# georghess/neurad-studio

Hardware: AMD Instinct MI355X
Metric: ray-samples/sec (4096 rays x 128 samples) (higher is better)
Workload: dtype f32; 1 GPU; BASELINE config[1]: NeuRAD hash-grid (16 levels, T=2^19, F=2, fp32) + 64-wide MLPs, 4096 rays x 128 samples per GPU, PowerSampler bins + ray ordering pass + fused field + compositing (forward / render path); rays_per_gpu=4096, samples_per_ray=128, parallelism=rays sharded x1, no collective

## Files before the change

neurad_studio_amd/csrc/render.hip:

```cpp
#include "common.h"
#include "render_variants.h"

namespace nrhip {

struct FieldDev {
  GridDev grid;
  const void* table;
  float scale;
  const float* gw0; const float* gb0;
  const float* gw1; const float* gb1;
  const float* fw0; const float* fb0;
  const float* fw1; const float* fb1;
  const float* fw2; const float* fb2;
  int use_sdf;
  float beta;
  uint32_t lay[NRHIP_MAX_LEVELS * 4];
};

struct SaveDev {
  float* enc;
  float* hg;
  float* xf;
  float* hf;
};

template <int H, Prod PROD = Prod::F32>
struct Lds {
  static constexpr int NB = H / 16;
  static constexpr int WS(int n) { return PROD == Prod::Bf16Split ? n + n / 2 : n; }
  static constexpr int G0 = 0;
  static constexpr int G1 = G0 + WS(H * 32);
  static constexpr int F0 = G1 + WS(32 * H);
  static constexpr int F1 = F0 + WS(H * 32);
  static constexpr int F2 = F1 + WS(H * H);
  static constexpr int SHW = F2 + 32 * H;
  static constexpr int SDFW = SHW + 16 * H;
  static constexpr int BG0 = SDFW + H;
  static constexpr int BG1 = BG0 + H;
  static constexpr int BF0 = BG1 + 36;
  static constexpr int BF1 = BF0 + H;
  static constexpr int BF2 = BF1 + H;
  static constexpr int SCAL = BF2 + 32;
  static constexpr int RB = SCAL + NRHIP_MAX_LEVELS;
  static constexpr int LAY = RB + 4 * H;
  static constexpr int FLG = LAY + 4 * NRHIP_MAX_LEVELS;
  static constexpr int TOTAL = FLG + 4;
  static constexpr int SHF = TOTAL;
  static constexpr int ASCAL = SHF + 16 * H;
  static constexpr int TOTAL_ACT = ASCAL + NRHIP_MAX_LEVELS;
};

struct ActorFieldDev {
  int K;
  int La;
  int log2T;
  float scale;
  float scal[NRHIP_MAX_LEVELS];
};

template <bool CHAIN, int NBLK, int NSTEP>
__device__ __forceinline__ float frag_src(const float* __restrict__ W, int ldw, int row_off, int e) {
  const int s3 = e & 3, lane = (e >> 2) & 63, rest = e >> 8;
  const int s4 = rest % (NSTEP / 4), mb = rest / (NSTEP / 4);
  const int s = 4 * s4 + s3, i = lane & 15, g = lane >> 4;
  const int col = CHAIN ? (16 * (s >> 2) + 4 * g + (s & 3)) : (8 * g + s);
  return W[(size_t)(row_off + 16 * mb + i) * ldw + col];
}

template <int L, int F>
struct EncFrame {
  static constexpr int LPL = (L + 3) / 4;
  static constexpr int W = LPL * F;
  static constexpr int NG = L / LPL;
  static constexpr int LF = L * F;
  static constexpr bool FULL = W == 8 && NG == 4;
  static_assert(W <= 8 && L % LPL == 0, "encoding frame: at most 8 features per lane group, whole levels per group");
  static __device__ __forceinline__ bool busy(int g) { return FULL || g < NG; }
};

template <int L, int F, int NBLK>
__device__ __forceinline__ float enc_frag_src(const float* __restrict__ W, int e) {
  using EF = EncFrame<L, F>;
  if constexpr (EF::FULL) {
    return frag_src<false, NBLK, 8>(W, EF::LF, 0, e);
  } else {
    const int s3 = e & 3, lane = (e >> 2) & 63, rest = e >> 8;
    const int s = 4 * (rest & 1) + s3, mb = rest >> 1, i = lane & 15, g = lane >> 4;
    return (s < EF::W && g < EF::NG) ? W[(size_t)(16 * mb + i) * EF::LF + EF::W * g + s] : 0.f;
  }
}

using bf16x4 = __attribute__((ext_vector_type(4))) short;

struct Split4 {
  bf16x4 h, m, l;
};

__device__ __forceinline__ uint32_t pack_hi16(uint32_t lo_src, uint32_t hi_src) {
  return __builtin_amdgcn_perm(hi_src, lo_src, 0x07060302u);
}

__device__ __forceinline__ Split4 split4(float x0, float x1, float x2, float x3) {
  const float x[4] = {x0, x1, x2, x3};
  uint32_t h[4], m[4], l[4];
#pragma unroll
  for (int k = 0; k < 4; ++k) {
    h[k] = __float_as_uint(x[k]) & 0xffff0000u;
    const float r1 = x[k] - __uint_as_float(h[k]);
    m[k] = __float_as_uint(r1) & 0xffff0000u;
    l[k] = __float_as_uint(r1 - __uint_as_float(m[k]));
  }
  Split4 s;
  s.h = __builtin_bit_cast(bf16x4, uint2{pack_hi16(h[0], h[1]), pack_hi16(h[2], h[3])});
  s.m = __builtin_bit_cast(bf16x4, uint2{pack_hi16(m[0], m[1]), pack_hi16(m[2], m[3])});
  s.l = __builtin_bit_cast(bf16x4, uint2{pack_hi16(l[0], l[1]), pack_hi16(l[2], l[3])});
  return s;
}

template <int NBLK, int KB>
__device__ __forceinline__ void mfma_layer_split(const float* __restrict__ wf, int lane, const float (&b)[4 * KB],
                                                 f32x4 (&acc)[NBLK]) {
  const uint2* w2 = reinterpret_cast<const uint2*>(wf);
  constexpr bool kTwoSets = NBLK < 4;
  f32x4 acc2[kTwoSets ? NBLK : 1];
  if constexpr (kTwoSets) {
#pragma unroll
    for (int mb = 0; mb < NBLK; ++mb) acc2[mb] = f32x4{0.f, 0.f, 0.f, 0.f};
  }
#pragma unroll
  for (int kb = 0; kb < KB; ++kb) {
    const Split4 x = split4(b[4 * kb], b[4 * kb + 1], b[4 * kb + 2], b[4 * kb + 3]);
    bf16x4 ah[NBLK], am[NBLK], al[NBLK];
#pragma unroll
    for (int mb = 0; mb < NBLK; ++mb) {
      const uint4 hm = reinterpret_cast<const uint4*>(wf)[(mb * KB + kb) * 64 + lane];
      ah[mb] = __builtin_bit_cast(bf16x4, uint2{hm.x, hm.y});
      am[mb] = __builtin_bit_cast(bf16x4, uint2{hm.z, hm.w});
      al[mb] = __builtin_bit_cast(bf16x4, w2[NBLK * KB * 128 + (mb * KB + kb) * 64 + lane]);
    }
#define NR_TERM(ACC, A_, X_)                                                                          \
  _Pragma("unroll") for (int mb = 0; mb < NBLK; ++mb) ACC[mb] =                                        \
      __builtin_amdgcn_mfma_f32_16x16x16bf16_1k(A_[mb], X_, ACC[mb], 0, 0, 0);
    if constexpr (kTwoSets) {
      NR_TERM(acc2, al, x.h) NR_TERM(acc, ah, x.h) NR_TERM(acc2, ah, x.l) NR_TERM(acc, ah, x.m)
      NR_TERM(acc2, am, x.m) NR_TERM(acc, am, x.h)
    } else {
      NR_TERM(acc, al, x.h) NR_TERM(acc, ah, x.l) NR_TERM(acc, am, x.m) NR_TERM(acc, am, x.h) NR_TERM(acc, ah, x.m)
      NR_TERM(acc, ah, x.h)
    }
#undef NR_TERM
  }
  if constexpr (kTwoSets) {
#pragma unroll
    for (int mb = 0; mb < NBLK; ++mb) acc[mb] += acc2[mb];
  }
}

template <bool CHAIN, int NBLK, int KB>
__device__ __forceinline__ void stage_split_matrix(float* __restrict__ dst, const float* __restrict__ W, int ldw,
                                                   int row_off) {
  unsigned short* d16 = reinterpret_cast<unsigned short*>(dst);
  for (int e = threadIdx.x; e < NBLK * KB * 64 * 4; e += 256) {
    const int v = e & 3, lane = (e >> 2) & 63, rest = e >> 8;
    const int kb = rest % KB, mb = rest / KB;
    const int i = lane & 15, g = lane >> 4;
    const int col = CHAIN ? (16 * kb + 4 * g + v) : (8 * g + 4 * kb + v);
    const float w = W[(size_t)(row_off + 16 * mb + i) * ldw + col];
    const uint32_t h = __float_as_uint(w) & 0xffff0000u;
    const float r1 = w - __uint_as_float(h);
    const uint32_t m = __float_as_uint(r1) & 0xffff0000u;
    const uint32_t l = __float_as_uint(r1 - __uint_as_float(m));
    const int blk = (mb * KB + kb) * 64 + lane;
    d16[blk * 8 + v] = (unsigned short)(h >> 16);
    d16[blk * 8 + 4 + v] = (unsigned short)(m >> 16);
    d16[NBLK * KB * 64 * 8 + blk * 4 + v] = (unsigned short)(l >> 16);
  }
}

using f16x8 = __attribute__((ext_vector_type(8))) _Float16;
using f16x2 = __attribute__((ext_vector_type(2))) _Float16;
using f32x2 = __attribute__((ext_vector_type(2))) float;
constexpr float kPairAct = 64.f, kPairW = 128.f, kPairFit = 65000.f;
constexpr bool kPairsDefault = true;

template <bool CHAIN, int NBLK, int KQ>
__device__ __forceinline__ float pair_src(const float* __restrict__ W, int ldw, int row_off, int e) {
  const int t = e & 7, lane = (e >> 3) & 63, rest = e >> 9;
  const int q = rest % KQ, mb = rest / KQ;
  const int i = lane & 15, g = lane >> 4;
  const int col = CHAIN ? (16 * (2 * q + (t >> 2)) + 4 * g + (t & 3)) : (8 * g + t);
  return W[(size_t)(row_off + 16 * mb + i) * ldw + col];
}
__device__ __forceinline__ bool pair_store(float* __restrict__ region, int N, int e, float w) {
  _Float16* d16 = reinterpret_cast<_Float16*>(region);
  const float ws = w * kPairW;
  const _Float16 h = (_Float16)ws;
  d16[e] = h;
  d16[N + e] = (_Float16)(ws - (float)h);
  return !(fabsf(ws) < kPairFit);
}

template <bool CHAIN, int NBLK, int KQ>
// ... 37 lines not shown
#pragma unroll
      for (int mb = 0; mb < NBLK; ++mb)
        acc[mb] = __builtin_amdgcn_mfma_f32_16x16x32_f16(w8[(mb * KQ + q) * 64 + lane], xl, acc[mb], 0, 0, 0);
    }
  }
#pragma unroll
  for (int mb = 0; mb < NBLK; ++mb) acc[mb] *= 1.f / kPairW;
}

template <Prod PROD, bool CHAIN, int NBLK, int K>
__device__ __forceinline__ void tile_layer(const float* __restrict__ wf, const float* __restrict__ W, int ldw, int row_off,
                                           bool wbad, int lane, const float (&b)[K], f32x4 (&acc)[NBLK]) {
  if constexpr (PROD == Prod::F16Pairs) mfma_layer_pairs<CHAIN, NBLK, K / 8>(wf, W, ldw, row_off, wbad, lane, b, acc);
  else if constexpr (PROD == Prod::Bf16Split) mfma_layer_split<NBLK, K / 4>(wf, lane, b, acc);
  else mfma_layer<NBLK, K>(wf, lane, b, acc);
}

template <int L, int F, int H, Prod PROD = Prod::F32>
__device__ __forceinline__ void stage_field_weights(const FieldDev& fd, float* __restrict__ lds) {
  using Ld = Lds<H, PROD>;
  constexpr int LF = EncFrame<L, F>::LF;
  static_assert(PROD == Prod::F32 || EncFrame<L, F>::FULL, "split / pair products: L * F == 32 only");
  constexpr int NB = H / 16;
  constexpr int T = 256;
  constexpr int N_G0 = H * 32 / T, N_G1 = 32 * H / T, N_F0 = H * 32 / T, N_F1 = H * H / T, N_F2 = 32 * H / T,
                N_SH = 16 * H / T;
  static_assert((H * 32) % T == 0 && (H * H) % T == 0 && (16 * H) % T == 0, "regions are whole passes of the block");
  const int tid = threadIdx.x;
  float vg0[N_G0], vg1[N_G1], vf0[N_F0], vf1[N_F1], vf2[N_F2], vsh[N_SH], vs[7];
  if constexpr (PROD == Prod::Bf16Split) {
    stage_split_matrix<false, NB, 2>(lds + Ld::G0, fd.gw0, LF, 0);
    stage_split_matrix<true, 2, NB>(lds + Ld::G1, fd.gw1, H, 1);
    stage_split_matrix<true, NB, 2>(lds + Ld::F0, fd.fw0, 48, 0);
    stage_split_matrix<true, NB, NB>(lds + Ld::F1, fd.fw1, H, 0);
  } else if constexpr (PROD == Prod::F16Pairs) {
    static_assert(H % 32 == 0, "fp16 pairs: K = 32 steps");
    if (tid == 0) reinterpret_cast<int*>(lds)[Ld::FLG] = 0;
    __syncthreads();
#pragma unroll
    for (int it = 0; it < N_G0; ++it) vg0[it] = pair_src<false, NB, 1>(fd.gw0, LF, 0, it * T + tid);
#pragma unroll
    for (int it = 0; it < N_G1; ++it) vg1[it] = pair_src<true, 2, H / 32>(fd.gw1, H, 1, it * T + tid);
#pragma unroll
    for (int it = 0; it < N_F0; ++it) vf0[it] = pair_src<true, NB, 1>(fd.fw0, 48, 0, it * T + tid);
#pragma unroll
    for (int it = 0; it < N_F1; ++it) vf1[it] = pair_src<true, NB, H / 32>(fd.fw1, H, 0, it * T + tid);
  } else {
#pragma unroll
    for (int it = 0; it < N_G0; ++it) vg0[it] = enc_frag_src<L, F, NB>(fd.gw0, it * T + tid);
#pragma unroll
    for (int it = 0; it < N_G1; ++it) vg1[it] = frag_src<true, 2, H / 4>(fd.gw1, H, 1, it * T + tid);
#pragma unroll
    for (int it = 0; it < N_F0; ++it) vf0[it] = frag_src<true, NB, 8>(fd.fw0, 48, 0, it * T + tid);
#pragma unroll
    for (int it = 0; it < N_F1; ++it) vf1[it] = frag_src<true, NB, H / 4>(fd.fw1, H, 0, it * T + tid);
  }
#pragma unroll
  for (int it = 0; it < N_F2; ++it) vf2[it] = frag_src<true, 2, H / 4>(fd.fw2, H, 0, it * T + tid);
#pragma unroll
  for (int it = 0; it < N_SH; ++it) {
    const int e = it * T + tid, c = e / H, n = e - c * H;
    vsh[it] = fd.fw0[(size_t)n * 48 + 32 + c];
  }
  const int th = tid < H ? tid : 0, t33 = tid < 33 ? tid : 0, t32 = tid & 31;
  vs[0] = fd.gw1[th];
  vs[1] = fd.gb0 ? fd.gb0[th] : 0.f;
  vs[2] = fd.fb0 ? fd.fb0[th] : 0.f;
  vs[3] = fd.fb1 ? fd.fb1[th] : 0.f;
  vs[4] = fd.gb1 ? fd.gb1[t33] : 0.f;
  vs[5] = fd.fb2 ? fd.fb2[t32] : 0.f;
  vs[6] = fd.grid.scal[t32];
  if constexpr (PROD == Prod::F16Pairs) {
    constexpr float kB = kPairAct * kPairW;
    vs[0] *= 1.f / kPairAct, vs[1] *= kB, vs[2] *= kB, vs[3] *= kB;
    if (t33 != 0) vs[4] *= kB;
#pragma unroll
    for (int it = 0; it < N_F2; ++it) vf2[it] *= 1.f / kPairAct;
#pragma unroll
    for (int it = 0; it < N_SH; ++it) vsh[it] *= kB;
    bool bad = false;
#pragma unroll
    for (int it = 0; it < N_G0; ++it) bad |= pair_store(lds + Ld::G0, H * 32, it * T + tid, vg0[it]);
#pragma unroll
    for (int it = 0; it < N_G1; ++it) bad |= pair_store(lds + Ld::G1, 32 * H, it * T + tid, vg1[it]);
#pragma unroll
    for (int it = 0; it < N_F0; ++it) bad |= pair_store(lds + Ld::F0, H * 32, it * T + tid, vf0[it]);
#pragma unroll
    for (int it = 0; it < N_F1; ++it) bad |= pair_store(lds + Ld::F1, H * H, it * T + tid, vf1[it]);
    if (bad) reinterpret_cast<int*>(lds)[Ld::FLG] = 1;
  }
  if constexpr (PROD == Prod::F32) {
#pragma unroll
    for (int it = 0; it < N_G0; ++it) lds[Ld::G0 + it * T + tid] = vg0[it];
#pragma unroll
    for (int it = 0; it < N_G1; ++it) lds[Ld::G1 + it * T + tid] = vg1[it];
#pragma unroll
    for (int it = 0; it < N_F0; ++it) lds[Ld::F0 + it * T + tid] = vf0[it];
#pragma unroll
    for (int it = 0; it < N_F1; ++it) lds[Ld::F1 + it * T + tid] = vf1[it];
  }
#pragma unroll
  for (int it = 0; it < N_F2; ++it) lds[Ld::F2 + it * T + tid] = vf2[it];
#pragma unroll
  for (int it = 0; it < N_SH; ++it) lds[Ld::SHW + it * T + tid] = vsh[it];
  if (tid < H) {
    lds[Ld::SDFW + tid] = vs[0];
    lds[Ld::BG0 + tid] = vs[1];
    lds[Ld::BF0 + tid] = vs[2];
    lds[Ld::BF1 + tid] = vs[3];
  }
  if (tid < 33) lds[Ld::BG1 + tid] = vs[4];
  if (tid < 32) {
    lds[Ld::BF2 + tid] = vs[5];
    lds[Ld::SCAL + tid] = vs[6];
  }
}

__device__ __forceinline__ void stream_store(float* p, f32x4 v) { __builtin_nontemporal_store(v, reinterpret_cast<f32x4*>(p)); }

template <int N>
__device__ __forceinline__ float row_shr(float v, float fill) {
  return dpp_row_shr<N>(v, fill);
}
__device__ __forceinline__ float row_sum16(float v) {
  v += __shfl_xor(v, 1, 64);
  v += __shfl_xor(v, 2, 64);
  v += __shfl_xor(v, 4, 64);
  v += __shfl_xor(v, 8, 64);
  return v;
}

template <int LPL, int F>
struct TileFetch {
  float fv[LPL][8][F];
  float x, y, z, std;
  float t0, t1;
};

struct RayRange {
  int64_t end;
  int S, stride;
};

struct PendingTile {
  int64_t pos;
  int64_t ray;
  int t;
  bool valid;
  float t0, t1;
  float ox, oy, oz, dx, dy, dz, area;
  int ncand;
};

__device__ __forceinline__ void load_pending(PendingTile& p, int64_t pos, int t, const RayRange& rr, int j,
                                             const int32_t* __restrict__ order, const float* __restrict__ ro,
                                             const float* __restrict__ rd, const float* __restrict__ rarea,
                                             const float* __restrict__ rstarts, const float* __restrict__ rends,
                                             const int32_t* __restrict__ cand_count = nullptr) {
  p.pos = pos, p.t = t, p.valid = pos < rr.end;
  const int64_t pc = p.valid ? pos : rr.end - 1;
  const int64_t ray = order ? (int64_t)order[pc] : pc;
  p.ray = ray;
  const int s = p.valid ? 16 * t + j : j;
  const int64_t si = ray * rr.stride + (s < rr.S ? s : rr.S - 1);
  p.t0 = rstarts[si];
  p.t1 = rends[si];
  p.ox = ro[3 * ray], p.oy = ro[3 * ray + 1], p.oz = ro[3 * ray + 2];
  p.dx = rd[3 * ray], p.dy = rd[3 * ray + 1], p.dz = rd[3 * ray + 2];
  p.area = rarea[ray];
  p.ncand = cand_count ? cand_count[ray] : 0;
}

__device__ __forceinline__ void load_pending_packed(PendingTile& p, int64_t pos, int t, const RayRange& rr, int j,
                                                    const int32_t* __restrict__ order, const float* __restrict__ ro,
                                                    const float* __restrict__ rd, const float* __restrict__ rarea,
                                                    const float* __restrict__ rstarts, const float* __restrict__ rends,
                                                    const int64_t* __restrict__ segs, int& first, int& count,
                                                    const int32_t* __restrict__ cand_count = nullptr) {
  p.pos = pos, p.t = t, p.valid = pos < rr.end;
  const int64_t pc = p.valid ? pos : rr.end - 1;
  const int64_t ray = order ? (int64_t)order[pc] : pc;
  p.ray = ray;
  const int b = (int)segs[ray], n = (int)segs[ray + 1] - b;
  first = b, count = n;
  const int s = p.valid ? 16 * t + j : j;
  int si = b + (s < n ? s : n - 1);
  si = si < 0 ? 0 : si;
  si = si < rr.S ? si : rr.S - 1;
  p.t0 = rstarts[si];
  p.t1 = rends[si];
  p.ox = ro[3 * ray], p.oy = ro[3 * ray + 1], p.oz = ro[3 * ray + 2];
  p.dx = rd[3 * ray], p.dy = rd[3 * ray + 1], p.dz = rd[3 * ray + 2];
  p.area = rarea[ray];
  p.ncand = cand_count ? cand_count[ray] : 0;
}

__device__ __forceinline__ void layout_corners(float x, float y, float z, float scale, uint32_t my, uint32_t mz,
                                               uint32_t mask, uint32_t (&idx)[8]) {
  const float sx = __fmul_rn(x, scale), sy = __fmul_rn(y, scale), sz = __fmul_rn(z, scale);
  const uint32_t ifx = (uint32_t)(int)floorf(sx), ify = (uint32_t)(int)floorf(sy), ifz = (uint32_t)(int)floorf(sz);
  const uint32_t icx = (uint32_t)(int)ceilf(sx), icy = (uint32_t)(int)ceilf(sy), icz = (uint32_t)(int)ceilf(sz);
  const uint32_t hyc = icy * my, hyf = ify * my, hzc = icz * mz, hzf = ifz * mz;
  idx[0] = (icx ^ hyc ^ hzc) & mask;
  idx[1] = (icx ^ hyf ^ hzc) & mask;
  idx[2] = (ifx ^ hyf ^ hzc) & mask;
  idx[3] = (ifx ^ hyc ^ hzc) & mask;
  idx[4] = (icx ^ hyc ^ hzf) & mask;
  idx[5] = (icx ^ hyf ^ hzf) & mask;
  idx[6] = (ifx ^ hyf ^ hzf) & mask;
  idx[7] = (ifx ^ hyc ^ hzf) & mask;
}

template <int L, int F, bool HALF, bool RELAY = false>
__device__ __forceinline__ void issue_tile(const FieldDev& fd, const PendingTile& pt, int g, uint32_t mask,
                                           const float* scal_lds, TileFetch<EncFrame<L, F>::LPL, F>& tf,
                                           const uint32_t* lay_lds = nullptr) {
  constexpr int LPL = EncFrame<L, F>::LPL;
  tf.t0 = pt.t0;
  tf.t1 = pt.t1;
  const SamplePos p = sample_position(pt.ox, pt.oy, pt.oz, pt.dx, pt.dy, pt.dz, pt.area, pt.t0, pt.t1, fd.scale);
  tf.x = p.x, tf.y = p.y, tf.z = p.z, tf.std = p.std;
  if (!EncFrame<L, F>::busy(g)) return;
#pragma unroll
  for (int q = 0; q < LPL; ++q) {
    if constexpr (RELAY) {
      const uint4 ly = *reinterpret_cast<const uint4*>(lay_lds + 4 * q);
      uint32_t idx[8];
      layout_corners(p.x, p.y, p.z, scal_lds[q], ly.x, ly.y, ly.z, idx);
#pragma unroll
      for (int k = 0; k < 8; ++k) Entry<F, HALF>::load(fd.table, ly.w + idx[k], tf.fv[q][k]);
    } else {
      const Corners cs = hash_corners(p.x, p.y, p.z, scal_lds[q], mask);
#pragma unroll
      for (int k = 0; k < 8; ++k)
        Entry<F, HALF>::load(fd.table, ((uint32_t)(LPL * g + q) << fd.grid.log2T) + cs.idx[k], tf.fv[q][k]);
    }
  }
}

template <int L, int F, bool HALF>
__device__ __forceinline__ void issue_tile_actors(const FieldDev& fd, const ActorFieldDev& ad, const PendingTile& pt, int g,
                                                  uint32_t mask, const float* scal_lds, const float* ascal_lds,
                                                  const int32_t* __restrict__ cand_actor,
                                                  const float* __restrict__ cand_w2b, const float* __restrict__ bounds,
                                                  const void* const* __restrict__ tables,
                                                  TileFetch<EncFrame<L, F>::LPL, F>& tf, int& slot_out) {
  constexpr int LPL = EncFrame<L, F>::LPL;
  const bool busy = EncFrame<L, F>::busy(g);
  const int n = __builtin_amdgcn_readfirstlane(pt.ncand);
  const uint32_t row = (uint32_t)__builtin_amdgcn_readfirstlane((int)((uint32_t)pt.ray * (uint32_t)ad.K));
  int slot = -1;
  if (n > 0) {
    const SamplePos gs = sample_gaussian(pt.ox, pt.oy, pt.oz, pt.dx, pt.dy, pt.dz, pt.area, pt.t0, pt.t1);
    for (int c = 0; c < n; ++c) {
      const float* w = cand_w2b + (row + (uint32_t)c) * 12u;
      const int act = cand_actor[row + (uint32_t)c];
      const float bx = w[0] * gs.x + w[1] * gs.y + w[2] * gs.z + w[3];
      const float by = w[4] * gs.x + w[5] * gs.y + w[6] * gs.z + w[7];
      const float bz = w[8] * gs.x + w[9] * gs.y + w[10] * gs.z + w[11];
      if (fabsf(bx) < bounds[3 * act] && fabsf(by) < bounds[3 * act + 1] && fabsf(bz) < bounds[3 * act + 2]) slot = c;
    }
  }
  slot_out = slot;
  tf.t0 = pt.t0;
  tf.t1 = pt.t1;
  unsigned long long todo = __ballot(slot >= 0);
  const SamplePos gs = sample_gaussian(pt.ox, pt.oy, pt.oz, pt.dx, pt.dy, pt.dz, pt.area, pt.t0, pt.t1);
  const uint32_t amask = (1u << ad.log2T) - 1u;
  while (todo) {
    const int c = __builtin_amdgcn_readlane(slot, (int)__builtin_ctzll(todo));
    const bool mine = slot == c;
    todo &= ~__ballot(mine);
    const float* w = cand_w2b + (row + (uint32_t)c) * 12u;
    const int act = cand_actor[row + (uint32_t)c];
    const void* tb = tables[act];
    if (mine) {
      const float bx = w[0] * gs.x + w[1] * gs.y + w[2] * gs.z + w[3];
      const float by = w[4] * gs.x + w[5] * gs.y + w[6] * gs.z + w[7];
      const float bz = w[8] * gs.x + w[9] * gs.y + w[10] * gs.z + w[11];
      const SamplePos p = contract_gaussian(bx, by, bz, gs.std, ad.scale);
      tf.x = p.x, tf.y = p.y, tf.z = p.z, tf.std = p.std;
      if (busy) {
#pragma unroll
        for (int q = 0; q < LPL; ++q) {
          const int lv = LPL * g + q, alv = lv < ad.La ? lv : ad.La - 1;
          const Corners cs = hash_corners(p.x, p.y, p.z, ascal_lds[alv], amask);
#pragma unroll
          for (int k = 0; k < 8; ++k) Entry<F, HALF>::load(tb, ((uint32_t)alv << ad.log2T) + cs.idx[k], tf.fv[q][k]);
        }
      }
    }
  }
  if (slot < 0) {
    const SamplePos p = contract_gaussian(gs.x, gs.y, gs.z, gs.std, fd.scale);
    tf.x = p.x, tf.y = p.y, tf.z = p.z, tf.std = p.std;
    if (busy) {
#pragma unroll
      for (int q = 0; q < LPL; ++q) {
        const Corners cs = hash_corners(p.x, p.y, p.z, scal_lds[q], mask);
#pragma unroll
        for (int k = 0; k < 8; ++k)
          Entry<F, HALF>::load(fd.table, ((uint32_t)(LPL * g + q) << fd.grid.log2T) + cs.idx[k], tf.fv[q][k]);
      }
    }
  }
}

__device__ __forceinline__ void actor_tile_sh(int slot, uint32_t row, int g, float dx, float dy, float dz,
                                              const float* __restrict__ cand_w2b, float (&shb)[4]) {
  float bx = dx, by = dy, bz = dz;
  unsigned long long todo = __ballot(slot >= 0);
  while (todo) {
    const int c = __builtin_amdgcn_readlane(slot, (int)__builtin_ctzll(todo));
    const bool mine = slot == c;
    todo &= ~__ballot(mine);
    const float* w = cand_w2b + (row + (uint32_t)c) * 12u;
    const float ddx = w[0] * dx + w[1] * dy + w[2] * dz;
    const float ddy = w[4] * dx + w[5] * dy + w[6] * dz;
    const float ddz = w[8] * dx + w[9] * dy + w[10] * dz;
    const float nn = sqrtf(ddx * ddx + ddy * ddy + ddz * ddz) + 1e-7f;
    if (mine) bx = ddx / nn, by = ddy / nn, bz = ddz / nn;
  }
  float sh[16];
  sh4((bx + 1.f) / 2.f, (by + 1.f) / 2.f, (bz + 1.f) / 2.f, sh);
#pragma unroll
  for (int c = 0; c < 16; ++c)
    if ((c >> 2) == g) shb[c & 3] = sh[c];
}

template <int L, int F>
__device__ __forceinline__ void blend_tile_actors(const TileFetch<EncFrame<L, F>::LPL, F>& tf, int slot, int g, int La,
                                                  const float* scal_lds, const float* ascal_lds, float (&feat)[8]) {
  using EF = EncFrame<L, F>;
  constexpr int LPL = EF::LPL;
  const bool in_box = slot >= 0;
#pragma unroll
  for (int q = 0; q < LPL; ++q) {
    const int lv = LPL * g + q, alv = lv < La ? lv : La - 1;
    const float sc = in_box ? ascal_lds[alv] : scal_lds[q];
    Corners c;
    const float sx = __fmul_rn(tf.x, sc), sy = __fmul_rn(tf.y, sc), sz = __fmul_rn(tf.z, sc);
    c.ox = __fsub_rn(sx, floorf(sx)), c.oy = __fsub_rn(sy, floorf(sy)), c.oz = __fsub_rn(sz, floorf(sz));
    float v[F];
    lerp_corners<F>(c, tf.fv[q], v);
    const float rw = (in_box && lv >= La) ? 0.f : rescale_weight(sc, tf.std);
#pragma unroll
    for (int f = 0; f < F; ++f) feat[q * F + f] = EF::busy(g) ? v[f] * rw : 0.f;
  }
#pragma unroll
  for (int k = EF::W; k < 8; ++k) feat[k] = 0.f;
}

template <int L, int F>
__device__ __forceinline__ void blend_tile(const TileFetch<EncFrame<L, F>::LPL, F>& tf, int g, const float* scal_lds,
                                           float (&feat)[8]) {
  using EF = EncFrame<L, F>;
  constexpr int LPL = EF::LPL;
#pragma unroll
  for (int q = 0; q < LPL; ++q) {
    const float sc = scal_lds[q];
    Corners c;
    const float sx = __fmul_rn(tf.x, sc), sy = __fmul_rn(tf.y, sc), sz = __fmul_rn(tf.z, sc);
    c.ox = __fsub_rn(sx, floorf(sx)), c.oy = __fsub_rn(sy, floorf(sy)), c.oz = __fsub_rn(sz, floorf(sz));
    float v[F];
    lerp_corners<F>(c, tf.fv[q], v);
    const float rw = rescale_weight(sc, tf.std);
#pragma unroll
    for (int f = 0; f < F; ++f) feat[q * F + f] = EF::busy(g) ? v[f] * rw : 0.f;
  }
#pragma unroll
  for (int k = EF::W; k < 8; ++k) feat[k] = 0.f;
}

template <int L, int F, int H, bool HALF, Out OUT, Src SRC, Prod PROD, Lay LAY = Lay::Dense>
__global__ __launch_bounds__(256, 2) void render_kernel(
    FieldDev fd, int64_t n_rays, int S, int stride, const int32_t* __restrict__ order, const float* __restrict__ ro,
    const float* __restrict__ rd, const float* __restrict__ rarea, const float* __restrict__ rstarts,
    const float* __restrict__ rends, float* __restrict__ out_feat, float* __restrict__ out_depth,
    float* __restrict__ out_acc, float* __restrict__ out_w, float* __restrict__ out_sdf, float* __restrict__ out_alpha,
    SaveDev sv, float stop_eps, const int32_t* __restrict__ range, ActorFieldDev ad,
    const int32_t* __restrict__ cand_count,
    const int32_t* __restrict__ cand_actor, const float* __restrict__ cand_w2b, const float* __restrict__ bounds,
    const void* const* __restrict__ tables) {
  using EF = EncFrame<L, F>;
  static_assert(render_variant_ok(L, F, OUT, SRC, PROD, LAY), "not a legal variant: see render_variant_ok");
  static_assert(H % 16 == 0 && H >= 16 && H <= 128, "hidden width");
  constexpr bool COMPOSITE = OUT == Out::Composite;
  constexpr bool ACT = SRC == Src::Actors, RELAY = SRC == Src::EvalTable, OVR = SRC == Src::Overrides;
  constexpr bool PAIRS = PROD == Prod::F16Pairs;
  constexpr bool PACKED = LAY != Lay::Dense;
  const int64_t* const segs = LAY == Lay::PackedActors ? reinterpret_cast<const int64_t*>(sv.enc)
                                                       : reinterpret_cast<const int64_t*>(tables);
  const int32_t* const pcand = ACT ? cand_count : nullptr;
  const int32_t* const ovr_row = cand_count;
  const float* const ovr_rows = cand_w2b;
  const float* const ovr_dirs = bounds;
  using Ld = Lds<H, PROD>;
  constexpr int NB = H / 16;
  constexpr int LPL = EF::LPL;
  constexpr bool DEFER = COMPOSITE;
  extern __shared__ __attribute__((aligned(16))) float lds[];

  stage_field_weights<L, F, H, PROD>(fd, lds);
  if constexpr (ACT || OVR) {
    for (int e = threadIdx.x; e < 16 * H; e += 256) lds[Ld::SHF + e] = frag_src<true, NB, 4>(fd.fw0 + 32, 48, 0, e);
  }
  if constexpr (ACT) {
    if (threadIdx.x < ad.La) lds[Ld::ASCAL + threadIdx.x] = ad.scal[threadIdx.x];
  }
  if constexpr (RELAY) {
    if (threadIdx.x < 4 * L) reinterpret_cast<uint32_t*>(lds + Ld::LAY)[threadIdx.x] = fd.lay[threadIdx.x];
  }
  __syncthreads();
  bool wbad = false;
  if constexpr (PAIRS) wbad = __builtin_amdgcn_readfirstlane(reinterpret_cast<const int*>(lds)[Ld::FLG]) != 0;

  const int lane = threadIdx.x & 63;
  const int wid = __builtin_amdgcn_readfirstlane(threadIdx.x >> 6);
  const int j = lane & 15, g = lane >> 4;
  const uint32_t mask = (1u << fd.grid.log2T) - 1u;
  const int ntile = (S + 15) >> 4;

  const int nx = (int)gridDim.x < 8 ? (int)gridDim.x : 8;
  const int xcd = (int)blockIdx.x % nx, lb = (int)blockIdx.x / nx;
  const int nblk = ((int)gridDim.x - xcd + nx - 1) / nx;
  const int64_t first = range ? range[0] : 0, count = range ? range[1] - range[0] : n_rays;
  const int64_t lo = first + count * xcd / nx;
  const RayRange rr{first + count * (xcd + 1) / nx, S, stride};
  const int64_t pos_step = (int64_t)nblk * 4;

  const float* scal_l = lds + Ld::SCAL + LPL * g;
  const uint32_t* lay_l = reinterpret_cast<const uint32_t*>(lds + Ld::LAY) + 4 * LPL * g;
  float* rbw = lds + Ld::RB + wid * H;
  int64_t pos = lo + (int64_t)lb * 4 + wid;
  if (pos >= rr.end) return;
  int t = 0;
  TileFetch<LPL, F> tf;
  if constexpr (!EF::FULL) tf = TileFetch<LPL, F>{};
  int ta = -1;
  const float* ascal_l = lds + Ld::ASCAL;
  PendingTile q;
  int qb = 0, qn = 0;
  auto tiles_of = [](int n) { return n > 16 ? (n + 15) >> 4 : 1; };
  if constexpr (PACKED) load_pending_packed(q, pos, 0, rr, j, order, ro, rd, rarea, rstarts, rends, segs, qb, qn, pcand);
  else load_pending(q, pos, 0, rr, j, order, ro, rd, rarea, rstarts, rends, cand_count);
  int64_t ray = q.ray;
  int cb = 0, cn = 0;
  if constexpr (PACKED) cb = qb, cn = qn;
  if constexpr (ACT) issue_tile_actors<L, F, HALF>(fd, ad, q, g, mask, scal_l, ascal_l, cand_actor, cand_w2b, bounds, tables, tf, ta);
  else issue_tile<L, F, HALF, RELAY>(fd, q, g, mask, scal_l, tf, lay_l);
  if constexpr (OVR && PACKED) ta = (q.valid && j < qn && qb + j >= 0 && qb + j < S) ? ovr_row[qb + j] : -1;
  else if constexpr (OVR) ta = (q.valid && j < S) ? ovr_row[q.ray * S + j] : -1;
  {
    const bool wrap = (PACKED ? tiles_of(cn) : ntile) == 1;
    if constexpr (PACKED) load_pending_packed(q, wrap ? pos + pos_step : pos, wrap ? 0 : 1, rr, j, order, ro, rd, rarea, rstarts, rends, segs, qb, qn, pcand);
    else load_pending(q, wrap ? pos + pos_step : pos, wrap ? 0 : 1, rr, j, order, ro, rd, rarea, rstarts, rends, cand_count);
  }

  f32x4 shq = f32x4{0.f, 0.f, 0.f, 0.f};
  float carry = 0.f, acc_w = 0.f, acc_d = 0.f;
  constexpr int NHA = DEFER ? H / 4 : 1;
  float ha[NHA];
  f32x4 fa[2];

  while (true) {
    if (t == 0) {
      const float dx = rd[3 * ray], dy = rd[3 * ray + 1], dz = rd[3 * ray + 2];
      float sh[16];
      sh4((dx + 1.f) / 2.f, (dy + 1.f) / 2.f, (dz + 1.f) / 2.f, sh);
      if constexpr (!COMPOSITE) {
#pragma unroll
        for (int c = 0; c < 16; ++c)
          if ((c >> 2) == g) shq[c & 3] = sh[c];
      }
      f32x4 rb[NB];
#pragma unroll
      for (int mb = 0; mb < NB; ++mb) rb[mb] = *reinterpret_cast<const f32x4*>(lds + Ld::BF0 + 16 * mb + 4 * g);
#pragma unroll
      for (int c = 0; c < 16; ++c)
#pragma unroll
        for (int mb = 0; mb < NB; ++mb) {
          const f32x4 w = *reinterpret_cast<const f32x4*>(lds + Ld::SHW + c * H + 16 * mb + 4 * g);
#pragma unroll
          for (int r = 0; r < 4; ++r) rb[mb][r] = fmaf(w[r], sh[c], rb[mb][r]);
        }
#pragma unroll
      for (int mb = 0; mb < NB; ++mb) *reinterpret_cast<f32x4*>(rbw + 16 * mb + 4 * g) = rb[mb];
      carry = COMPOSITE ? (fd.use_sdf ? 1.f : 0.f) : 0.f;
      acc_w = 0.f, acc_d = 0.f;
      fa[0] = fa[1] = f32x4{0.f, 0.f, 0.f, 0.f};
#pragma unroll
      for (int k = 0; k < NHA; ++k) ha[k] = 0.f;
    }

    int opaque = 0;
    asm volatile("" : "+v"(opaque));
    const float* lw = lds + opaque;
    const int s = 16 * t + j;
    const bool live = s < (PACKED ? cn : S);
    const float t0 = tf.t0, t1 = tf.t1;

    float feat[8];
    bool tile_hit = false;
    float shb[4] = {0.f, 0.f, 0.f, 0.f};
    if constexpr (ACT) {
      blend_tile_actors<L, F>(tf, ta, g, ad.La, scal_l, ascal_l, feat);
      tile_hit = __ballot(ta >= 0) != 0ull;
      if (tile_hit)
        actor_tile_sh(ta, (uint32_t)__builtin_amdgcn_readfirstlane((int)((uint32_t)ray * (uint32_t)ad.K)), g, rd[3 * ray],
                      rd[3 * ray + 1], rd[3 * ray + 2], cand_w2b, shb);
    } else {
      blend_tile<L, F>(tf, g, scal_l, feat);
      if constexpr (PAIRS) {
#pragma unroll
        for (int k = 0; k < 8; ++k) feat[k] *= kPairAct;
      }
      if constexpr (OVR) {
        tile_hit = __ballot(ta >= 0) != 0ull;
        if (tile_hit) {
          float bx = rd[3 * ray], by = rd[3 * ray + 1], bz = rd[3 * ray + 2];
          if (ta >= 0) {
            const float* rp = ovr_rows + (size_t)ta * EF::LF + EF::W * g;
            if constexpr (EF::FULL) {
              const f32x4 r0 = *reinterpret_cast<const f32x4*>(rp), r1 = *reinterpret_cast<const f32x4*>(rp + 4);
#pragma unroll
              for (int k = 0; k < 4; ++k) feat[k] = r0[k], feat[4 + k] = r1[k];
            } else if (EF::busy(g)) {
#pragma unroll
              for (int k = 0; k < EF::W; ++k) feat[k] = rp[k];
            }
            bx = ovr_dirs[3 * (size_t)ta], by = ovr_dirs[3 * (size_t)ta + 1], bz = ovr_dirs[3 * (size_t)ta + 2];
          }
          float sh[16];
          sh4((bx + 1.f) / 2.f, (by + 1.f) / 2.f, (bz + 1.f) / 2.f, sh);
#pragma unroll
          for (int c = 0; c < 16; ++c)
            if ((c >> 2) == g) shb[c & 3] = sh[c];
        }
      }
    }
    __builtin_amdgcn_sched_barrier(0);

    bool stop_here = false;
    if constexpr (COMPOSITE) {
      if (stop_eps > 0.f) {
        const float c = __builtin_bit_cast(float, __builtin_amdgcn_readfirstlane(__builtin_bit_cast(int, carry)));
        stop_here = fd.use_sdf ? (c < stop_eps) : (c > -__logf(stop_eps));
      }
    }
    const bool last_tile = t == (PACKED ? tiles_of(cn) : ntile) - 1;
    const bool ray_done = last_tile || stop_here;

    if (ray_done && q.valid && q.pos == pos) {
      if constexpr (PACKED) load_pending_packed(q, pos + pos_step, 0, rr, j, order, ro, rd, rarea, rstarts, rends, segs, qb, qn, pcand);
      else load_pending(q, pos + pos_step, 0, rr, j, order, ro, rd, rarea, rstarts, rends, cand_count);
    }
    const bool have_next = q.valid;
    const int64_t npos = q.pos, nray = q.ray;
    const int nt = q.t;
    int nb = 0, nn = 0;
    if constexpr (PACKED) nb = qb, nn = qn;
    if constexpr (ACT) issue_tile_actors<L, F, HALF>(fd, ad, q, g, mask, scal_l, ascal_l, cand_actor, cand_w2b, bounds, tables, tf, ta);
    else issue_tile<L, F, HALF, RELAY>(fd, q, g, mask, scal_l, tf, lay_l);
    if constexpr (OVR && PACKED) {
      const int s2 = 16 * q.t + j;
      ta = (q.valid && s2 < qn && qb + s2 >= 0 && qb + s2 < S) ? ovr_row[qb + s2] : -1;
    } else if constexpr (OVR) {
      ta = (q.valid && 16 * q.t + j < S) ? ovr_row[q.ray * S + 16 * q.t + j] : -1;
    }
    {
      const bool wrap = nt + 1 == (PACKED ? tiles_of(nn) : ntile);
      if constexpr (PACKED)
        load_pending_packed(q, wrap ? npos + pos_step : npos, wrap ? 0 : nt + 1, rr, j, order, ro, rd, rarea, rstarts, rends, segs, qb, qn, pcand);
      else
        load_pending(q, wrap ? npos + pos_step : npos, wrap ? 0 : nt + 1, rr, j, order, ro, rd, rarea, rstarts, rends,
                     cand_count);
    }
    __builtin_amdgcn_sched_barrier(0);

    if constexpr (PACKED) {
      if (cn <= 0) {
        if (COMPOSITE && j == 0) {
          float* fp = out_feat + ray * 32;
          *reinterpret_cast<f32x4*>(fp + 4 * g) = f32x4{0.f, 0.f, 0.f, 0.f};
          *reinterpret_cast<f32x4*>(fp + 16 + 4 * g) = f32x4{0.f, 0.f, 0.f, 0.f};
          if (g == 0) {
            out_acc[ray] = 0.f;
            out_depth[ray] = 0.f;
          }
        }
        if (!have_next) break;
        pos = npos, ray = nray, t = nt, cb = nb, cn = nn;
        continue;
      }
    }

    bool saving = false;
    int64_t srow = 0;
    if constexpr (!COMPOSITE) {
      saving = sv.enc != nullptr && live;
      srow = PACKED ? (int64_t)cb + s : ray * S + s;
      if (saving) {
        constexpr float u = PAIRS ? 1.f / kPairAct : 1.f;
        float* ep = sv.enc + srow * EF::LF + EF::W * g;
        if constexpr (EF::FULL) {
          stream_store(ep, f32x4{feat[0] * u, feat[1] * u, feat[2] * u, feat[3] * u});
          stream_store(ep + 4, f32x4{feat[4] * u, feat[5] * u, feat[6] * u, feat[7] * u});
        } else if (EF::busy(g)) {
          if constexpr (EF::W == 4) {
            stream_store(ep, f32x4{feat[0] * u, feat[1] * u, feat[2] * u, feat[3] * u});
          } else {
#pragma unroll
            for (int k = 0; k < EF::W; ++k) __builtin_nontemporal_store(feat[k] * u, ep + k);
          }
        }
      }
    }

    f32x4 h[NB];
#pragma unroll
    for (int mb = 0; mb < NB; ++mb) h[mb] = *reinterpret_cast<const f32x4*>(lw + Ld::BG0 + 16 * mb + 4 * g);
    tile_layer<PROD, false>(lw + Ld::G0, fd.gw0, EF::LF, 0, wbad, lane, feat, h);
    float hb[H / 4];
#pragma unroll
    for (int mb = 0; mb < NB; ++mb)
#pragma unroll
      for (int r = 0; r < 4; ++r) hb[4 * mb + r] = fmaxf(h[mb][r], 0.f);

    if constexpr (!COMPOSITE) {
      if (saving) {
        constexpr float u = PAIRS ? 1.f / kPairAct : 1.f;
#pragma unroll
        for (int mb = 0; mb < NB; ++mb)
          stream_store(sv.hg + srow * H + 16 * mb + 4 * g,
                       f32x4{hb[4 * mb] * u, hb[4 * mb + 1] * u, hb[4 * mb + 2] * u, hb[4 * mb + 3] * u});
      }
    }

    float sdf = 0.f;
#pragma unroll
    for (int mb = 0; mb < NB; ++mb) {
      const f32x4 w = *reinterpret_cast<const f32x4*>(lw + Ld::SDFW + 16 * mb + 4 * g);
#pragma unroll
      for (int r = 0; r < 4; ++r) sdf = fmaf(w[r], hb[4 * mb + r], sdf);
    }
    sdf += __shfl_xor(sdf, 16, 64);
    sdf += __shfl_xor(sdf, 32, 64);
    sdf += lw[Ld::BG1];
    f32x4 e[2];
#pragma unroll
    for (int mb = 0; mb < 2; ++mb) {
      const float* bp = lw + Ld::BG1 + 1 + 16 * mb + 4 * g;
      e[mb] = f32x4{bp[0], bp[1], bp[2], bp[3]};
    }
    tile_layer<PROD, true>(lw + Ld::G1, fd.gw1, H, 1, wbad, lane, hb, e);
    float eb[8];
#pragma unroll
    for (int k = 0; k < 8; ++k) eb[k] = e[k >> 2][k & 3];

    if constexpr (!COMPOSITE) {
      if (saving) {
        constexpr float u = PAIRS ? 1.f / kPairAct : 1.f;
        float* xp = sv.xf + srow * 48;
        stream_store(xp + 4 * g, e[0] * u);
        stream_store(xp + 16 + 4 * g, e[1] * u);
        stream_store(xp + 32 + 4 * g, tile_hit ? f32x4{shb[0], shb[1], shb[2], shb[3]} : shq);
      }
    }
    if (!tile_hit) {
#pragma unroll
      for (int mb = 0; mb < NB; ++mb) h[mb] = *reinterpret_cast<const f32x4*>(lw + Ld::RB + wid * H + 16 * mb + 4 * g);
    } else {
#pragma unroll
      for (int mb = 0; mb < NB; ++mb) h[mb] = *reinterpret_cast<const f32x4*>(lw + Ld::BF0 + 16 * mb + 4 * g);
      mfma_layer<NB, 4>(lw + Ld::SHF, lane, shb, h);
    }
    tile_layer<PROD, true>(lw + Ld::F0, fd.fw0, 48, 0, wbad, lane, eb, h);
#pragma unroll
    for (int mb = 0; mb < NB; ++mb)
#pragma unroll
      for (int r = 0; r < 4; ++r) hb[4 * mb + r] = fmaxf(h[mb][r], 0.f);
    if constexpr (!COMPOSITE) {
      if (saving) {
        constexpr float u = PAIRS ? 1.f / kPairAct : 1.f;
#pragma unroll
        for (int mb = 0; mb < NB; ++mb)
          stream_store(sv.hf + srow * (2 * H) + 16 * mb + 4 * g,
                       f32x4{hb[4 * mb] * u, hb[4 * mb + 1] * u, hb[4 * mb + 2] * u, hb[4 * mb + 3] * u});
      }
    }
#pragma unroll
    for (int mb = 0; mb < NB; ++mb) h[mb] = *reinterpret_cast<const f32x4*>(lw + Ld::BF1 + 16 * mb + 4 * g);
    tile_layer<PROD, true>(lw + Ld::F1, fd.fw1, H, 0, wbad, lane, hb, h);
#pragma unroll
    for (int mb = 0; mb < NB; ++mb)
#pragma unroll
      for (int r = 0; r < 4; ++r) hb[4 * mb + r] = fmaxf(h[mb][r], 0.f);
    if constexpr (!COMPOSITE) {
      if (saving) {
        constexpr float u = PAIRS ? 1.f / kPairAct : 1.f;
#pragma unroll
        for (int mb = 0; mb < NB; ++mb)
          stream_store(sv.hf + srow * (2 * H) + H + 16 * mb + 4 * g,
                       f32x4{hb[4 * mb] * u, hb[4 * mb + 1] * u, hb[4 * mb + 2] * u, hb[4 * mb + 3] * u});
      }
    }

    float a_or_d;
    if (fd.use_sdf) a_or_d = __builtin_amdgcn_rcpf(1.f + __expf(sdf * fd.beta));
    else a_or_d = expf(sdf);

    if constexpr (!COMPOSITE) {
      f32x4 o[2];
#pragma unroll
      for (int mb = 0; mb < 2; ++mb) o[mb] = *reinterpret_cast<const f32x4*>(lw + Ld::BF2 + 16 * mb + 4 * g);
      mfma_layer<2, H / 4>(lw + Ld::F2, lane, hb, o);
      if constexpr (PAIRS) {
        o[0] += e[0] * (1.f / kPairAct);
        o[1] += e[1] * (1.f / kPairAct);
      } else {
        o[0] += e[0];
        o[1] += e[1];
      }
      if (live) {
        const int64_t si = PACKED ? (int64_t)cb + s : ray * S + s;
        float* fp = out_feat + si * 32;
        stream_store(fp + 4 * g, o[0]);
        stream_store(fp + 16 + 4 * g, o[1]);
// ... 506 lines not shown
```

Baseline: 3.613 billion ray-samples/s.

## Compute sample positions once per 64-sample block and share via LDS

```diff
diff --git a/neurad_studio_amd/csrc/render.hip b/neurad_studio_amd/csrc/render.hip
--- a/neurad_studio_amd/csrc/render.hip
+++ b/neurad_studio_amd/csrc/render.hip
@@ -24,6 +24,7 @@
   float* hf;
 };
 
+constexpr int kBlockGeo = 4 * 64;
 template <int H, Prod PROD = Prod::F32>
 struct Lds {
   static constexpr int NB = H / 16;
@@ -44,10 +45,12 @@
   static constexpr int RB = SCAL + NRHIP_MAX_LEVELS;
   static constexpr int LAY = RB + 4 * H;
   static constexpr int FLG = LAY + 4 * NRHIP_MAX_LEVELS;
-  static constexpr int TOTAL = FLG + 4;
+  static constexpr int GEO = FLG + 4;
+  static constexpr int TOTAL = GEO + 4 * kBlockGeo;
   static constexpr int SHF = TOTAL;
   static constexpr int ASCAL = SHF + 16 * H;
-  static constexpr int TOTAL_ACT = ASCAL + NRHIP_MAX_LEVELS;
+  static constexpr int AGEO = ASCAL + NRHIP_MAX_LEVELS;
+  static constexpr int TOTAL_ACT = AGEO + 4 * kBlockGeo;
 };
 
 struct ActorFieldDev {
@@ -391,7 +394,30 @@
   int ncand;
 };
 
-__device__ __forceinline__ void load_pending(PendingTile& p, int64_t pos, int t, const RayRange& rr, int j,
+__device__ __forceinline__ float from_lane(float v, int byte_addr) {
+  return __builtin_bit_cast(float, __builtin_amdgcn_ds_bpermute(byte_addr, __builtin_bit_cast(int, v)));
+}
+__device__ __forceinline__ void put_block(float* geo, int lane, const SamplePos& p) {
+  geo[lane] = p.x, geo[64 + lane] = p.y, geo[128 + lane] = p.z, geo[192 + lane] = p.std;
+}
+__device__ __forceinline__ SamplePos get_block(const float* geo, int src) {
+  SamplePos p;
+  p.x = geo[src], p.y = geo[64 + src], p.z = geo[128 + src], p.std = geo[192 + src];
+  return p;
+}
+
+template <bool ACT>
+__device__ __forceinline__ void fill_block(float* geo, float* ageo, int lane, const PendingTile& pt, float scale) {
+  if constexpr (ACT) {
+    const SamplePos gs = sample_gaussian(pt.ox, pt.oy, pt.oz, pt.dx, pt.dy, pt.dz, pt.area, pt.t0, pt.t1);
+    put_block(ageo, lane, gs);
+    put_block(geo, lane, contract_gaussian(gs.x, gs.y, gs.z, gs.std, scale));
+  } else {
+    put_block(geo, lane, sample_position(pt.ox, pt.oy, pt.oz, pt.dx, pt.dy, pt.dz, pt.area, pt.t0, pt.t1, scale));
+  }
+}
+
+__device__ __forceinline__ void load_pending(PendingTile& p, int64_t pos, int t, const RayRange& rr, int lane,
                                              const int32_t* __restrict__ order, const float* __restrict__ ro,
                                              const float* __restrict__ rd, const float* __restrict__ rarea,
                                              const float* __restrict__ rstarts, const float* __restrict__ rends,
@@ -400,17 +426,19 @@
   const int64_t pc = p.valid ? pos : rr.end - 1;
   const int64_t ray = order ? (int64_t)order[pc] : pc;
   p.ray = ray;
-  const int s = p.valid ? 16 * t + j : j;
+  const int s = p.valid ? 64 * (t >> 2) + lane : lane;
   const int64_t si = ray * rr.stride + (s < rr.S ? s : rr.S - 1);
-  p.t0 = rstarts[si];
-  p.t1 = rends[si];
+  if ((t & 3) == 0) {
+    p.t0 = rstarts[si];
+    p.t1 = rends[si];
+  }
   p.ox = ro[3 * ray], p.oy = ro[3 * ray + 1], p.oz = ro[3 * ray + 2];
   p.dx = rd[3 * ray], p.dy = rd[3 * ray + 1], p.dz = rd[3 * ray + 2];
   p.area = rarea[ray];
   p.ncand = cand_count ? cand_count[ray] : 0;
 }
 
-__device__ __forceinline__ void load_pending_packed(PendingTile& p, int64_t pos, int t, const RayRange& rr, int j,
+__device__ __forceinline__ void load_pending_packed(PendingTile& p, int64_t pos, int t, const RayRange& rr, int lane,
                                                     const int32_t* __restrict__ order, const float* __restrict__ ro,
                                                     const float* __restrict__ rd, const float* __restrict__ rarea,
                                                     const float* __restrict__ rstarts, const float* __restrict__ rends,
@@ -422,12 +450,14 @@
   p.ray = ray;
   const int b = (int)segs[ray], n = (int)segs[ray + 1] - b;
   first = b, count = n;
-  const int s = p.valid ? 16 * t + j : j;
+  const int s = p.valid ? 64 * (t >> 2) + lane : lane;
   int si = b + (s < n ? s : n - 1);
   si = si < 0 ? 0 : si;
   si = si < rr.S ? si : rr.S - 1;
-  p.t0 = rstarts[si];
-  p.t1 = rends[si];
+  if ((t & 3) == 0) {
+    p.t0 = rstarts[si];
+    p.t1 = rends[si];
+  }
   p.ox = ro[3 * ray], p.oy = ro[3 * ray + 1], p.oz = ro[3 * ray + 2];
   p.dx = rd[3 * ray], p.dy = rd[3 * ray + 1], p.dz = rd[3 * ray + 2];
   p.area = rarea[ray];
@@ -453,12 +483,13 @@
 template <int L, int F, bool HALF, bool RELAY = false>
 __device__ __forceinline__ void issue_tile(const FieldDev& fd, const PendingTile& pt, int g, uint32_t mask,
                                            const float* scal_lds, TileFetch<EncFrame<L, F>::LPL, F>& tf,
-                                           const uint32_t* lay_lds = nullptr) {
+                                           float* geo, int lane, const uint32_t* lay_lds = nullptr) {
   constexpr int LPL = EncFrame<L, F>::LPL;
-  tf.t0 = pt.t0;
-  tf.t1 = pt.t1;
-  const SamplePos p = sample_position(pt.ox, pt.oy, pt.oz, pt.dx, pt.dy, pt.dz, pt.area, pt.t0, pt.t1, fd.scale);
-  tf.x = p.x, tf.y = p.y, tf.z = p.z, tf.std = p.std;
+  if ((pt.t & 3) == 0) fill_block<false>(geo, nullptr, lane, pt, fd.scale);
+  const int src = 16 * (pt.t & 3) + (lane & 15);
+  const SamplePos p = get_block(geo, src);
+  tf.t0 = from_lane(pt.t0, src << 2);
+  tf.t1 = from_lane(pt.t1, src << 2);
   if (!EncFrame<L, F>::busy(g)) return;
 #pragma unroll
   for (int q = 0; q < LPL; ++q) {
@@ -483,14 +514,19 @@
                                                   const int32_t* __restrict__ cand_actor,
                                                   const float* __restrict__ cand_w2b, const float* __restrict__ bounds,
                                                   const void* const* __restrict__ tables,
-                                                  TileFetch<EncFrame<L, F>::LPL, F>& tf, int& slot_out) {
+                                                  TileFetch<EncFrame<L, F>::LPL, F>& tf, int& slot_out,
+                                                  float* geo, float* ageo, int lane) {
   constexpr int LPL = EncFrame<L, F>::LPL;
   const bool busy = EncFrame<L, F>::busy(g);
   const int n = __builtin_amdgcn_readfirstlane(pt.ncand);
   const uint32_t row = (uint32_t)__builtin_amdgcn_readfirstlane((int)((uint32_t)pt.ray * (uint32_t)ad.K));
+  if ((pt.t & 3) == 0) fill_block<true>(geo, ageo, lane, pt, fd.scale);
+  const int src = 16 * (pt.t & 3) + (lane & 15);
+  const SamplePos gs = get_block(ageo, src), ps = get_block(geo, src);
+  tf.t0 = from_lane(pt.t0, src << 2);
+  tf.t1 = from_lane(pt.t1, src << 2);
   int slot = -1;
   if (n > 0) {
-    const SamplePos gs = sample_gaussian(pt.ox, pt.oy, pt.oz, pt.dx, pt.dy, pt.dz, pt.area, pt.t0, pt.t1);
     for (int c = 0; c < n; ++c) {
       const float* w = cand_w2b + (row + (uint32_t)c) * 12u;
       const int act = cand_actor[row + (uint32_t)c];
@@ -501,10 +537,7 @@
     }
   }
   slot_out = slot;
-  tf.t0 = pt.t0;
-  tf.t1 = pt.t1;
   unsigned long long todo = __ballot(slot >= 0);
-  const SamplePos gs = sample_gaussian(pt.ox, pt.oy, pt.oz, pt.dx, pt.dy, pt.dz, pt.area, pt.t0, pt.t1);
   const uint32_t amask = (1u << ad.log2T) - 1u;
   while (todo) {
     const int c = __builtin_amdgcn_readlane(slot, (int)__builtin_ctzll(todo));
@@ -531,7 +564,7 @@
     }
   }
   if (slot < 0) {
-    const SamplePos p = contract_gaussian(gs.x, gs.y, gs.z, gs.std, fd.scale);
+    const SamplePos p = ps;
     tf.x = p.x, tf.y = p.y, tf.z = p.z, tf.std = p.std;
     if (busy) {
 #pragma unroll
@@ -591,19 +624,19 @@
 }
 
 template <int L, int F>
-__device__ __forceinline__ void blend_tile(const TileFetch<EncFrame<L, F>::LPL, F>& tf, int g, const float* scal_lds,
-                                           float (&feat)[8]) {
+__device__ __forceinline__ void blend_tile(const TileFetch<EncFrame<L, F>::LPL, F>& tf, const SamplePos& p, int g,
+                                           const float* scal_lds, float (&feat)[8]) {
   using EF = EncFrame<L, F>;
   constexpr int LPL = EF::LPL;
 #pragma unroll
   for (int q = 0; q < LPL; ++q) {
     const float sc = scal_lds[q];
     Corners c;
-    const float sx = __fmul_rn(tf.x, sc), sy = __fmul_rn(tf.y, sc), sz = __fmul_rn(tf.z, sc);
+    const float sx = __fmul_rn(p.x, sc), sy = __fmul_rn(p.y, sc), sz = __fmul_rn(p.z, sc);
     c.ox = __fsub_rn(sx, floorf(sx)), c.oy = __fsub_rn(sy, floorf(sy)), c.oz = __fsub_rn(sz, floorf(sz));
     float v[F];
     lerp_corners<F>(c, tf.fv[q], v);
-    const float rw = rescale_weight(sc, tf.std);
+    const float rw = rescale_weight(sc, p.std);
 #pragma unroll
     for (int f = 0; f < F; ++f) feat[q * F + f] = EF::busy(g) ? v[f] * rw : 0.f;
   }
@@ -679,21 +712,23 @@
   int ta = -1;
   const float* ascal_l = lds + Ld::ASCAL;
   PendingTile q;
+  float* geo_w = lds + Ld::GEO + wid * kBlockGeo;
+  float* ageo_w = lds + (ACT ? Ld::AGEO : Ld::GEO) + wid * kBlockGeo;
   int qb = 0, qn = 0;
   auto tiles_of = [](int n) { return n > 16 ? (n + 15) >> 4 : 1; };
-  if constexpr (PACKED) load_pending_packed(q, pos, 0, rr, j, order, ro, rd, rarea, rstarts, rends, segs, qb, qn, pcand);
-  else load_pending(q, pos, 0, rr, j, order, ro, rd, rarea, rstarts, rends, cand_count);
+  if constexpr (PACKED) load_pending_packed(q, pos, 0, rr, lane, order, ro, rd, rarea, rstarts, rends, segs, qb, qn, pcand);
+  else load_pending(q, pos, 0, rr, lane, order, ro, rd, rarea, rstarts, rends, cand_count);
   int64_t ray = q.ray;
   int cb = 0, cn = 0;
   if constexpr (PACKED) cb = qb, cn = qn;
-  if constexpr (ACT) issue_tile_actors<L, F, HALF>(fd, ad, q, g, mask, scal_l, ascal_l, cand_actor, cand_w2b, bounds, tables, tf, ta);
-  else issue_tile<L, F, HALF, RELAY>(fd, q, g, mask, scal_l, tf, lay_l);
+  if constexpr (ACT) issue_tile_actors<L, F, HALF>(fd, ad, q, g, mask, scal_l, ascal_l, cand_actor, cand_w2b, bounds, tables, tf, ta, geo_w, ageo_w, lane);
+  else issue_tile<L, F, HALF, RELAY>(fd, q, g, mask, scal_l, tf, geo_w, lane, lay_l);
   if constexpr (OVR && PACKED) ta = (q.valid && j < qn && qb + j >= 0 && qb + j < S) ? ovr_row[qb + j] : -1;
   else if constexpr (OVR) ta = (q.valid && j < S) ? ovr_row[q.ray * S + j] : -1;
   {
     const bool wrap = (PACKED ? tiles_of(cn) : ntile) == 1;
-    if constexpr (PACKED) load_pending_packed(q, wrap ? pos + pos_step : pos, wrap ? 0 : 1, rr, j, order, ro, rd, rarea, rstarts, rends, segs, qb, qn, pcand);
-    else load_pending(q, wrap ? pos + pos_step : pos, wrap ? 0 : 1, rr, j, order, ro, rd, rarea, rstarts, rends, cand_count);
+    if constexpr (PACKED) load_pending_packed(q, wrap ? pos + pos_step : pos, wrap ? 0 : 1, rr, lane, order, ro, rd, rarea, rstarts, rends, segs, qb, qn, pcand);
+    else load_pending(q, wrap ? pos + pos_step : pos, wrap ? 0 : 1, rr, lane, order, ro, rd, rarea, rstarts, rends, cand_count);
   }
 
   f32x4 shq = f32x4{0.f, 0.f, 0.f, 0.f};
@@ -749,7 +784,7 @@
         actor_tile_sh(ta, (uint32_t)__builtin_amdgcn_readfirstlane((int)((uint32_t)ray * (uint32_t)ad.K)), g, rd[3 * ray],
                       rd[3 * ray + 1], rd[3 * ray + 2], cand_w2b, shb);
     } else {
-      blend_tile<L, F>(tf, g, scal_l, feat);
+      blend_tile<L, F>(tf, get_block(geo_w, 16 * (t & 3) + j), g, scal_l, feat);
       if constexpr (PAIRS) {
 #pragma unroll
         for (int k = 0; k < 8; ++k) feat[k] *= kPairAct;
@@ -791,16 +826,16 @@
     const bool ray_done = last_tile || stop_here;
 
     if (ray_done && q.valid && q.pos == pos) {
-      if constexpr (PACKED) load_pending_packed(q, pos + pos_step, 0, rr, j, order, ro, rd, rarea, rstarts, rends, segs, qb, qn, pcand);
-      else load_pending(q, pos + pos_step, 0, rr, j, order, ro, rd, rarea, rstarts, rends, cand_count);
+      if constexpr (PACKED) load_pending_packed(q, pos + pos_step, 0, rr, lane, order, ro, rd, rarea, rstarts, rends, segs, qb, qn, pcand);
+      else load_pending(q, pos + pos_step, 0, rr, lane, order, ro, rd, rarea, rstarts, rends, cand_count);
     }
     const bool have_next = q.valid;
     const int64_t npos = q.pos, nray = q.ray;
     const int nt = q.t;
     int nb = 0, nn = 0;
     if constexpr (PACKED) nb = qb, nn = qn;
-    if constexpr (ACT) issue_tile_actors<L, F, HALF>(fd, ad, q, g, mask, scal_l, ascal_l, cand_actor, cand_w2b, bounds, tables, tf, ta);
-    else issue_tile<L, F, HALF, RELAY>(fd, q, g, mask, scal_l, tf, lay_l);
+    if constexpr (ACT) issue_tile_actors<L, F, HALF>(fd, ad, q, g, mask, scal_l, ascal_l, cand_actor, cand_w2b, bounds, tables, tf, ta, geo_w, ageo_w, lane);
+    else issue_tile<L, F, HALF, RELAY>(fd, q, g, mask, scal_l, tf, geo_w, lane, lay_l);
     if constexpr (OVR && PACKED) {
       const int s2 = 16 * q.t + j;
       ta = (q.valid && s2 < qn && qb + s2 >= 0 && qb + s2 < S) ? ovr_row[qb + s2] : -1;
@@ -810,9 +845,9 @@
     {
       const bool wrap = nt + 1 == (PACKED ? tiles_of(nn) : ntile);
       if constexpr (PACKED)
-        load_pending_packed(q, wrap ? npos + pos_step : npos, wrap ? 0 : nt + 1, rr, j, order, ro, rd, rarea, rstarts, rends, segs, qb, qn, pcand);
+        load_pending_packed(q, wrap ? npos + pos_step : npos, wrap ? 0 : nt + 1, rr, lane, order, ro, rd, rarea, rstarts, rends, segs, qb, qn, pcand);
       else
-        load_pending(q, wrap ? npos + pos_step : npos, wrap ? 0 : nt + 1, rr, j, order, ro, rd, rarea, rstarts, rends,
+        load_pending(q, wrap ? npos + pos_step : npos, wrap ? 0 : nt + 1, rr, lane, order, ro, rd, rarea, rstarts, rends,
                      cand_count);
     }
     __builtin_amdgcn_sched_barrier(0);
```

After: 3.746 billion ray-samples/s (median of 6 runs). +3.7%, better.
